# project-codeflare/instaslice

Measured on NVIDIA B200. Metric: placements_per_sec, higher is better.
Workload: dtype u8

## Files before the change

instaslice_b200/csrc/isl_kernels.cuh:

```cuda
#pragma once

#include <cuda_runtime.h>
#include <stdint.h>

#include "../../include/islplace.h"

namespace isl {

constexpr uint32_t kChunk = 65536;
constexpr uint32_t kTile = 1024;
constexpr uint32_t kTileThreads = 256;
constexpr uint32_t kTilesPerChunk = kChunk / kTile;
constexpr uint32_t kQPad = 32;
constexpr uint32_t kQCap = kChunk + kQPad * ISL_MAX_PROFILES;
constexpr uint32_t kSweepThreads = 256;
constexpr uint32_t kSweepPerThread = 16;
constexpr uint32_t kSweepBlock = kSweepThreads * kSweepPerThread;
constexpr uint32_t kSkip = 0xFFu;
constexpr uint32_t kInf = 0xFFFFFFFFu;
constexpr uint32_t kMaxCand = ISL_MAX_PROFILES * ISL_MAX_STARTS;
constexpr uint32_t kChainThreads = 256;
constexpr uint32_t kMaxTables = ISL_MAX_TABLES;

#ifndef ISL_UNIFORM_WARP
// ... 871 lines not shown
    asm volatile("ld.relaxed.gpu.global.u64 %0, [%1];" : "=l"(v) : "l"(p) : "memory");
    return v;
}
__device__ __forceinline__ void st_relaxed_gpu_u64(unsigned long long* p, unsigned long long v) {
    asm volatile("st.relaxed.gpu.global.u64 [%0], %1;" ::"l"(p), "l"(v) : "memory");
}
__device__ __forceinline__ unsigned long long ld_relaxed_sys_u64(const unsigned long long* p) {
    unsigned long long v;
    asm volatile("ld.relaxed.sys.global.u64 %0, [%1];" : "=l"(v) : "l"(p) : "memory");
    return v;
}
__device__ __forceinline__ void st_relaxed_sys_u64(unsigned long long* p, unsigned long long v) {
    asm volatile("st.relaxed.sys.global.u64 [%0], %1;" ::"l"(p), "l"(v) : "memory");
}

__device__ __forceinline__ uint32_t spec_spread_warp(uint32_t h, uint32_t qc, uint32_t w, uint32_t members, int d, bool weighted, uint32_t lane) {
    const bool in = (members >> lane) & 1u;
    if (!weighted) w = 1;
    const uint32_t light = __ballot_sync(0xFFFFFFFFu, in && w <= 1), heavy = __ballot_sync(0xFFFFFFFFu, in && w > 1);
    const uint32_t tot = __reduce_add_sync(0xFFFFFFFFu, in ? qc * w : 0u);
    if (d == 0 || members == 0) return h;
    const uint32_t last = 31u - __clz(light ? light : heavy);
    int dp = in && lane != last && tot ? __float2int_rn((float)d * (float)qc / (float)tot) : 0;
    const int used = __reduce_add_sync(0xFFFFFFFFu, dp * (int)w);
    const int wl = (int)__shfl_sync(0xFFFFFFFFu, w, last);
    if (lane == last) dp = (d - used) / wl;
    if (!in) return h;
    const int v = (int)h + dp;
    return (uint32_t)(v < 0 ? 0 : (v > (int)qc ? (int)qc : v));
}

__device__ __forceinline__ uint32_t lds_u32(uint32_t sa) { uint32_t v; asm volatile("ld.shared.u32 %0, [%1];" : "=r"(v) : "r"(sa)); return v; }
__device__ __forceinline__ uint32_t lds_u16(uint32_t sa) { uint32_t v; asm volatile("ld.shared.u16 %0, [%1];" : "=r"(v) : "r"(sa)); return v; }
__device__ __forceinline__ void sts_v2_if(bool pred, uint32_t sa, uint32_t x, uint32_t y) {
    asm volatile("{ .reg .pred p; setp.ne.u32 p, %0, 0; @p st.shared.v2.u32 [%1], {%2, %3}; }" ::"r"((uint32_t)pred), "r"(sa), "r"(x), "r"(y) : "memory");
}
__device__ __forceinline__ uint32_t add_if(bool pred, uint32_t x, uint32_t inc) {
    asm volatile("{ .reg .pred p; setp.ne.u32 p, %1, 0; @p add.u32 %0, %0, %2; }" : "+r"(x) : "r"((uint32_t)pred), "r"(inc));
    return x;
}
__device__ __forceinline__ uint32_t redux_min_u32(uint32_t v) {
// ... 21 lines not shown
template <int K, bool kP15, bool kSpec>
__global__ void __launch_bounds__(kPipeThreads, 1) k_pipeline(CandTab tab, PipeArgs a) {
    extern __shared__ __align__(16) uint8_t smem[];
    uint32_t* s_occ32 = reinterpret_cast<uint32_t*>(smem);
    uint32_t* s_cand = reinterpret_cast<uint32_t*>(smem + kPipeOffCand);
    uint2* s_log = reinterpret_cast<uint2*>(smem + kPipeOffLog);
    __shared__ uint16_t s_feas[kMaxTables * 256];
    __shared__ uint8_t s_tab[kSegMax * kSubMax];
    __shared__ uint32_t s_heads[ISL_MAX_PROFILES], s_wn[ISL_MAX_PROFILES], s_wbase[ISL_MAX_PROFILES], s_qbeg[ISL_MAX_PROFILES], s_pop[ISL_MAX_PROFILES];
    __shared__ uint32_t s_maxacc[ISL_MAX_PROFILES], s_minsize[ISL_MAX_PROFILES], s_usable[kMaxTables], s_plist[ISL_MAX_PROFILES], s_nplist;
    __shared__ uint32_t s_warp[kPipeThreads / 32], s_ncand, s_nfree, s_nlog, s_idle, s_closed;
    __shared__ uint32_t s_specH[ISL_MAX_PROFILES], s_specX[ISL_MAX_PROFILES], s_specXp[ISL_MAX_PROFILES], s_qc[ISL_MAX_PROFILES];
    __shared__ uint32_t s_acc[4], s_grp_big, s_grp_small, s_specflag, s_bigd[32], s_nbigd, s_dqr[2], s_us[kMaxTables], s_qo[ISL_MAX_PROFILES];
    __shared__ uint8_t s_smallm[kMaxTables][ISL_MAX_PROFILES];
    __shared__ uint32_t s_wlo[ISL_MAX_PROFILES], s_wlen[ISL_MAX_PROFILES], s_woff[ISL_MAX_PROFILES], s_wvalid, s_restage;
    __shared__ uint32_t s_predc, s_predA[ISL_MAX_PROFILES], s_predB[ISL_MAX_PROFILES], s_havepred;
    __shared__ uint32_t s_Hc[ISL_MAX_PROFILES], s_Xc[ISL_MAX_PROFILES], s_capst[3], s_cap, s_capped;
    const uint32_t tid = threadIdx.x, lane = tid & 31u, warp = tid >> 5, seg = blockIdx.x;
    if (seg == a.n_seg) {
        __shared__ uint32_t s_stop;
        for (uint32_t c = 0; c < a.n_chunks; ++c) {
            if (tid == 0) {
                uint32_t stop = 0;
                const unsigned long long t0 = globaltimer_ns();
                while (ld_acquire_gpu(a.done_cnt + c) < a.n_seg) {
                    if (a.ready && ld_acquire_gpu(a.ready + (a.open ? c : a.chunks[c].batch)) == ~a.epoch) { stop = 1; break; }
                    __nanosleep(256);
                    if (globaltimer_ns() - t0 > a.wait_ns + 5000000000ull) __trap();
                }
                s_stop = stop;
            }
// ... 188 lines not shown
        auto pub_down = [&](unsigned long long* p, unsigned long long v) {
            st_relaxed_gpu_u64(p, v);
            if (xr) for (uint32_t r = a.spec_rank + 1; r < a.spec_world; ++r) st_relaxed_sys_u64(a.spec_peer[r] + (p - a.spec_mem), v);
        };
        auto pub_nb = [&](unsigned long long* p, unsigned long long v, bool prev) {
            const bool remote = xr && (prev ? (seg == 0 && a.spec_rank > 0) : (seg + 1 == a.n_seg && a.spec_rank + 1 < a.spec_world));
            if (remote) st_relaxed_sys_u64(a.spec_peer[prev ? a.spec_rank - 1 : a.spec_rank + 1] + (p - a.spec_mem), v);
            else st_relaxed_gpu_u64(p, v);
        };
        if (spec) {
            uint16_t* s_mj = reinterpret_cast<uint16_t*>(s_wkey);
            if (tid < ISL_MAX_PROFILES) {
                const bool on = ((active >> tid) & 1u) && s_maxacc[tid] != 0 && cc->qcnt[tid] != 0;
                s_qc[tid] = on ? cc->qcnt[tid] : 0u; s_qo[tid] = cc->qoff[tid];
                const uint32_t big = __ballot_sync(0xFFFFu, on && s_minsize[tid] >= 4), small = __ballot_sync(0xFFFFu, on && s_minsize[tid] < 4);
                if (tid == 0) { s_grp_big = big; s_grp_small = small; s_acc[0] = 0; s_acc[1] = 0; s_acc[2] = 0; }
                if (tid < kMaxTables) { uint32_t us = 0; for (uint32_t m = small; m; m &= m - 1) us |= s_smallm[tid][__ffs(m) - 1]; s_us[tid] = us; }
            }
            __syncthreads();
            {
                constexpr uint32_t kGpt = kSegMax / kPipeThreads;
                const uint32_t gb = s_grp_big, nb = s_nbigd;
                uint32_t mq = 0, mw = 0, mo = 0;
#pragma unroll
                for (uint32_t x = 0; x < kGpt; ++x) {
                    const uint32_t g = kGpt * tid + x;
                    if (g < n_sb) {
                        const uint32_t t = s_tab[sb_base + g], o0 = reinterpret_cast<const uint8_t*>(s_occ32)[sb_base + g], us = s_us[t];
                        uint32_t o = o0;
                        for (uint32_t it = 0; it < 2; ++it) {
                            uint32_t best = 0;
                            for (uint32_t y = 0; y < nb; ++y) {
// ... 34 lines not shown
                uint32_t ql = 0;
                for (uint32_t x = 0; x < kPer; ++x) { const uint32_t j = lane * kPer + x; if (j < gseg) ql += s_mj[j]; }
                uint32_t incl = ql;
#pragma unroll
                for (int d = 1; d < 32; d <<= 1) { const uint32_t t = __shfl_up_sync(0xFFFFFFFFu, incl, d); if ((int)lane >= d) incl += t; }
                uint32_t run = incl - ql, r = 0;
                for (uint32_t x = 0; x < kPer; ++x) {
                    const uint32_t j = lane * kPer + x;
                    if (j < gseg) { r += run < totb ? s_mj[kSpecStride + j] : s_mj[2 * kSpecStride + j]; run += s_mj[j]; }
                }
                r = __reduce_add_sync(0xFFFFFFFFu, r);
                const uint32_t Q = min(__shfl_sync(0xFFFFFFFFu, incl, 31), totb), R = min(r, tots);
                {
                    const uint32_t qcl = lane < ISL_MAX_PROFILES ? s_qc[lane] : 0u, wl = lane < ISL_MAX_PROFILES ? s_minsize[lane] : 1u;
                    uint32_t hg = lane < ISL_MAX_PROFILES && gseg == 0 && a.heads_in ? a.heads_in[(size_t)c * ISL_MAX_PROFILES + lane] : 0u;
                    if (gseg > 0) {
                        hg = spec_spread_warp(hg, qcl, wl, s_grp_big, (int)Q, false, lane);
                        hg = spec_spread_warp(hg, qcl, wl, s_grp_small, (int)R, true, lane);
                    }
                    if (lane < ISL_MAX_PROFILES) s_specH[lane] = hg;
                }
            }
            __syncthreads();
        }
        uint32_t rnd = 1;
        bool c_prev = spec ? gseg == 0 : seg == 0, need_sim = true, idle_break = false;
        bool known_exact = gseg == 0;
        if (tid == 0) { s_capst[0] = 0; s_capst[1] = 0; s_capst[2] = 0; s_cap = kLogCap + 1; s_capped = 0; s_wvalid = 0; s_havepred = 0; }
        bool p_final = false; unsigned long long p_word = 0;
        const unsigned long long t_cell = tr && spec ? globaltimer_ns() : 0ull, sims_cell = st_sims;
#ifdef ISL_SPEC_DBG_STAMPS
        unsigned long long* dbg = a.spec_dbg && a.spec_dbg_cell == ((c << 16) | seg) ? a.spec_dbg : nullptr;
#else
        constexpr unsigned long long* dbg = nullptr;
#endif
        while (true) {
        stamp_if(dbg && tid == 0, dbg + rnd * 8 + 0);
        if (need_sim) {
        asm volatile("cp.async.wait_group 0;" ::: "memory");
        if (tid < 32) {
            uint32_t h = 0, wn = 0, left = 0;
            bool from_done = false;
            const uint32_t tag = a.epoch & 0x7FFFu;
            stamp_if(tr && tid == 0, tr + 0);
            if (spec) {
                if (tid < ISL_MAX_PROFILES) h = s_specH[tid];
            } else if (sb > 0) {
                if (tid < ISL_MAX_PROFILES) h = s_heads[tid] + s_pop[tid];
            } else if (seg > 0) {
                const uint32_t* pt = a.tokens + (tok_chunk + seg - 1) * kTokStride + (tid & 15u);
                const uint32_t* pd = a.tokens + (tok_chunk + a.n_seg) * kTokStride + (tid & 15u);
                bool ok = tid >= ISL_MAX_PROFILES;
// ... 11 lines not shown
                const unsigned long long t0 = globaltimer_ns();
                while (!__all_sync(0xFFFFFFFFu, ok)) {
                    if (!ok) {
                        const uint32_t v = ld_relaxed_sys(slot);
                        if ((v >> 17) == xtag) { h = v & 0x1FFFFu; ok = true; }
                        else if (globaltimer_ns() - t0 > a.wait_ns) __trap();
                    }
                }
                if (tid < ISL_MAX_PROFILES) st_relaxed_sys(slot, 0u);
            } else if (tid < ISL_MAX_PROFILES) h = a.heads_in ? a.heads_in[(size_t)c * ISL_MAX_PROFILES + tid] : 0u;
            stamp_if(tr && tid == 0, tr + 1);
            const bool all_done = sb == 0 && __all_sync(0xFFFFFFFFu, from_done || tid >= ISL_MAX_PROFILES);
            if (tid < ISL_MAX_PROFILES) {
                const uint32_t qc = spec ? s_qc[tid] : cc->qcnt[tid], qo = spec ? s_qo[tid] : cc->qoff[tid];
                left = ((active >> tid) & 1u) && qc > h ? qc - h : 0u;
                wn = min(left, min(s_ncand * s_maxacc[tid], s_nfree / s_minsize[tid]));
                s_heads[tid] = h; s_pop[tid] = 0;
                if (!kSpec) {
                    s_wn[tid] = wn;
                    s_qbeg[tid] = qo + h;
                }
            }
            bool win_keep = true;
            if (kSpec) {
                uint32_t lo = 0, len = 0, woff = 0;
                bool ok = true;
                const uint32_t qc = tid < ISL_MAX_PROFILES ? s_qc[tid] : 0u;
                if (tid < ISL_MAX_PROFILES) {
                    lo = s_wlo[tid]; len = s_wlen[tid];
                    if (left == 0) woff = len;
                    else { ok = s_wvalid && h >= lo && (h + wn + 2 <= lo + len || lo + len >= qc); woff = h - lo; }
// ... 16 lines not shown
                if (kSpec) {
                    s_restage = win_keep ? 0u : 1u;
                    if (!win_keep) s_wvalid = idle ? 0u : 1u;
                }
                s_cap = spec && s_capst[1] && !known_exact ? min(kLogCap + 1, ((s_capst[0] * 21u) >> 4) + 64u) : kLogCap + 1;
                s_capped = 0;
            }
            uint32_t incl = wn + kWinPad;
#pragma unroll
            for (int d = 1; d < 16; d <<= 1) { const uint32_t t = __shfl_up_sync(0xFFFFFFFFu, incl, d); if ((int)lane >= d) incl += t; }
            if (tid < ISL_MAX_PROFILES) s_wbase[tid] = incl - (wn + kWinPad);
        }
        __syncthreads();
        stamp_if(tr && tid == 0, tr + 8);
        stamp_if(dbg && tid == 0, dbg + rnd * 8 + 1);
        if (s_idle && spec) { if (tid == 0) { s_nlog = 0; spec_steps = 0; spec_visited = 0; } }
        else if (s_idle) {
            if (warp == 0) {
                const bool last = seg == a.n_seg - 1;
                uint32_t* tok = a.tokens + (tok_chunk + seg) * kTokStride;
                uint32_t* peer = last && a.outbox ? a.outbox + (size_t)c * kTokStride : nullptr;
                if (lane < ISL_MAX_PROFILES) {
                    const uint32_t h = s_heads[lane];
                    st_relaxed_gpu(tok + lane, ((a.epoch & 0x7FFFu) << 17) | h);
                    if (last && a.heads_out) a.heads_out[(size_t)c * ISL_MAX_PROFILES + lane] = h;
                    if (peer) st_relaxed_sys(peer + lane, ((a.xepoch % 32767u + 1u) << 17) | h);
                }
                __syncwarp();
                if (lane == 0) {
                    if (tr) { tr[2] = globaltimer_ns(); tr[3] = tr[2]; }
// ... 3 lines not shown
            idle_break = true;
            break;
        }
        if (!s_idle) {
        {
            const uint32_t npl = kSpec && !s_restage ? 0u : s_nplist;
            const uint16_t* __restrict__ sq = reinterpret_cast<const uint16_t*>(smem + kPipeOffQ);
            for (uint32_t x = 0; x < npl; ++x) {
                const uint32_t p = s_plist[x], wn = kSpec ? s_wlen[p] : s_wn[p], pk = p << 11, qb = s_qbeg[p];
                uint32_t* __restrict__ dst = s_wkey + s_wbase[p];
                for (uint32_t i = tid; i < wn + kWinPad; i += kPipeThreads) { const uint32_t v = sq[qb + min(i, wn)]; dst[i] = i < wn ? (v << 15) | pk : kInf; }
            }
            stamp_if(tr && tid == 0, tr + 10);
            store_if(tr && tid == 0, tr + 11, s_wn[s_plist[0]] | ((unsigned long long)s_nfree << 32));
        }
        __syncthreads();
        stamp_if(tr && tid == 0, tr + 9);
        if (is_chain_warp(warp)) {
            const uint32_t n_cand = s_ncand;
            uint32_t tcur[K], tnext[K], tnn[K], wa[K], wa0[K];
#pragma unroll
            for (int k = 0; k < K; ++k) {
                wa0[k] = sa_wkey + 4 * (s_wbase[cprof[k]] + (kSpec ? s_woff[cprof[k]] : 0u));
                const bool has = valid[k];
                tcur[k] = has ? lds_u32(wa0[k]) | klow[k] : kInf;
                tnext[k] = has ? lds_u32(wa0[k] + 4) | klow[k] : kInf;
                const bool two = has && s_wn[cprof[k]] >= 1;
                tnn[k] = two ? lds_u32(wa0[k] + 8) : kInf;
                wa[k] = wa0[k] + 12;
            }
            uint32_t la = sa_log, ca = sa_cand + 8;
            uint32_t z0[K], z1[K], z2[K], g1[K], g2[K], cm8[K];
// ... 114 lines not shown
            const bool last = seg == a.n_seg - 1;
            uint32_t* peer = last && a.outbox ? a.outbox + (size_t)c * kTokStride : nullptr;
            if (last_sub && lane < ISL_MAX_PROFILES && !spec) {
                const uint32_t h = s_heads[lane] + s_pop[lane];
                st_relaxed_gpu(tok + lane, ((a.epoch & 0x7FFFu) << 17) | h);
                if (last && a.heads_out) a.heads_out[(size_t)c * ISL_MAX_PROFILES + lane] = h;
                if (peer) st_relaxed_sys(peer + lane, ((a.xepoch % 32767u + 1u) << 17) | h);
            }
            __syncwarp();
            if (lane == 0) {
                s_nlog = nlog;
                s_capped = cut ? 1u : 0u;
                if (tr) tr[2] = globaltimer_ns();
            }
        }
        else if (spec && tid == kPipeThreads - 32 && rnd >= 3 && gseg + 1 < gtot) {
            const unsigned long long t0 = globaltimer_ns();
            uint32_t spins = 0;
            while (true) {
                const unsigned long long w = sld(sm.ack + gseg + 1);
                if ((uint32_t)(w >> 32) == tage && (uint32_t)w + 2u >= rnd) break;
                if ((++spins & 255u) == 0 && globaltimer_ns() - t0 > a.wait_ns) __trap();
            }
        }
        }
        __syncthreads();
        }
        if (!spec) break;
        {
            const unsigned long long tagr = tagb | ((unsigned long long)rnd << 32);
            if (tid < 32) {
                uint32_t X = 0, dq = 0, dr = 0, pop = 0;
                const bool was_cut = s_capped != 0;
                if (tid < ISL_MAX_PROFILES) { pop = s_pop[tid]; X = s_heads[tid] + pop; }
                if (was_cut) {
                    int eq = 0, er = 0;
                    uint32_t xe = 0;
                    const uint32_t qcl = tid < ISL_MAX_PROFILES ? s_qc[tid] : 0u, wl = tid < ISL_MAX_PROFILES ? s_minsize[tid] : 1u;
                    if (tid < ISL_MAX_PROFILES) {
                        const int d = (int)s_heads[tid] - (int)s_Hc[tid];
                        if ((s_grp_big >> tid) & 1u) eq = d;
                        if ((s_grp_small >> tid) & 1u) er = d * (int)s_minsize[tid];
                        xe = s_Xc[tid];
                    }
                    eq = __reduce_add_sync(0xFFFFFFFFu, eq); er = __reduce_add_sync(0xFFFFFFFFu, er);
                    xe = spec_spread_warp(xe, qcl, wl, s_grp_big, eq, false, lane);
                    xe = spec_spread_warp(xe, qcl, wl, s_grp_small, er, true, lane);
                    if (tid < ISL_MAX_PROFILES) { X = max(xe, s_heads[tid]); pop = X - s_heads[tid]; }
                }
                if (tid < ISL_MAX_PROFILES) {
                    s_specX[tid] = X;
                    if (!was_cut) { s_Hc[tid] = s_heads[tid]; s_Xc[tid] = X; }
                    if ((s_grp_big >> tid) & 1u) dq = pop;
                    if ((s_grp_small >> tid) & 1u) dr = pop * s_minsize[tid];
                }
                if (tid == 0) { if (was_cut) s_capst[2] = 0; else { s_capst[0] = max(s_capst[0], s_nlog); s_capst[1] = 1; s_capst[2] = 1; } }
                dq = __reduce_add_sync(0xFFFFFFFFu, dq); dr = __reduce_add_sync(0xFFFFFFFFu, dr);
                if (rnd >= 3 && gseg + 1 < gtot && !(need_sim && !s_idle)) {
                    const unsigned long long t0 = globaltimer_ns();
                    uint32_t spins = 0;
                    while (true) {
                        const unsigned long long w = sld(sm.ack + gseg + 1);
                        if ((uint32_t)(w >> 32) == tage && (uint32_t)w + 2u >= rnd) break;
                        if ((++spins & 255u) == 0 && globaltimer_ns() - t0 > a.wait_ns) __trap();
                    }
                }
                if (tid < ISL_MAX_PROFILES) pub_nb(sm.x + ((size_t)gseg * 2 + (rnd & 1u)) * 16 + tid, tagr | X, false);
                if (tid == 16) pub_down(sm.d + (size_t)rnd * kSpecStride + gseg, tagr | ((c_prev ? 1u : 0u) << 31) | (dq << 13) | dr);
                if (tid == 0) { s_dqr[0] = dq; s_dqr[1] = dr; s_acc[0] = 0; s_acc[1] = 0; }
                stamp_if(dbg && tid == 0, dbg + rnd * 8 + 4);
            }
            __syncthreads();
            bool cbit = true;
            if (tid < gseg) {
                unsigned long long w = p_word;
                if (!p_final) {
                    const unsigned long long t0 = globaltimer_ns();
                    uint32_t spins = 0;
                    while (true) {
                        w = sld(sm.d + (size_t)rnd * kSpecStride + tid);
                        if ((w >> 32) == (tagr >> 32)) { cbit = (w >> 31) & 1u; break; }
                        if ((spins++ & 3u) == 0) {
                            w = sld(sm.df + tid);
                            if ((w >> 32) == (tagF >> 32) && ((w >> 24) & 0xFFu) <= rnd) { p_final = true; p_word = w; break; }
                        }
                        if ((spins & 255u) == 0 && globaltimer_ns() - t0 > a.wait_ns) __trap();
                    }
                }
                atomicAdd(&s_acc[0], (uint32_t)(w >> 13) & 0x7FFu);
                atomicAdd(&s_acc[1], (uint32_t)w & 0x1FFFu);
            }
            if (gseg > 0 && tid >= 192 && tid < 192 + ISL_MAX_PROFILES) {
                const uint32_t i = tid - 192;
                unsigned long long w = p_word;
                if (!p_final) {
                    const unsigned long long t0 = globaltimer_ns();
                    uint32_t spins = 0;
                    while (true) {
                        w = sld(sm.x + ((size_t)(gseg - 1) * 2 + (rnd & 1u)) * 16 + i);
                        if ((w >> 32) == (tagr >> 32)) break;
                        if ((spins++ & 3u) == 0) {
                            w = sld(sm.xf + (size_t)(gseg - 1) * 16 + i);
                            if ((w >> 32) == (tagF >> 32) && ((w >> 24) & 0xFFu) <= rnd) { p_final = true; p_word = w; break; }
                        }
                        if ((spins & 255u) == 0 && globaltimer_ns() - t0 > a.wait_ns) __trap();
                    }
                }
                s_specXp[i] = (uint32_t)w & 0x1FFFFu;
            }
            if (tid + 1 == gseg) s_predc = cbit ? 1u : 0u;
            const int unset = __syncthreads_count(!cbit);
            const bool allc = unset == 0;
            const bool near = allc || (unset == 1 && !s_predc);
            const bool certified = allc && c_prev;
            stamp_if(dbg && tid == 0, dbg + rnd * 8 + 5);
            store_if(dbg && tid == 0, dbg + rnd * 8 + 7, s_nlog | ((unsigned long long)need_sim << 32));
            if (gseg > 0 && tid == 192) pub_nb(sm.ack + gseg, ((unsigned long long)tage << 32) | (certified ? 0xFFFFu : rnd), true);
            if (certified) {
                if (tid < ISL_MAX_PROFILES) {
                    pub_nb(sm.xf + (size_t)gseg * 16 + tid, tagF | (rnd << 24) | s_specX[tid], false);
                    if (gseg == gtot - 1 && a.heads_out) a.heads_out[(size_t)c * ISL_MAX_PROFILES + tid] = s_specX[tid];
                }
                if (tid == 16) pub_down(sm.df + gseg, tagF | (rnd << 24) | (s_dqr[0] << 13) | s_dqr[1]);
                if (tid == 0) { st_steps += spec_steps; st_visited += spec_visited; if (gseg == gtot - 1) { st_rounds_sum += rnd; ++st_cells; } if (tr) { tr[0] = t_cell; tr[2] = globaltimer_ns(); tr[6] = s_nlog; tr[7] = st_sims - sims_cell; tr[11] = rnd; } }
                break;
            }
            if (tid < 32) {
                const bool same = tid >= ISL_MAX_PROFILES || s_specH[tid] == s_specXp[tid];
                const bool cnow = __all_sync(0xFFFFFFFFu, same);
                uint32_t mq = 0, mr = 0, hold = 0, hn = 0;
                const uint32_t qcl = tid < ISL_MAX_PROFILES ? s_qc[tid] : 0u, wl = tid < ISL_MAX_PROFILES ? s_minsize[tid] : 1u;
                if (tid < ISL_MAX_PROFILES) {
                    hold = s_specH[tid];
                    hn = s_specXp[tid];
                    if ((s_grp_big >> tid) & 1u) mq = hn;
                    if ((s_grp_small >> tid) & 1u) mr = hn * s_minsize[tid];
                }
                mq = __reduce_add_sync(0xFFFFFFFFu, mq); mr = __reduce_add_sync(0xFFFFFFFFu, mr);
                hn = spec_spread_warp(hn, qcl, wl, s_grp_big, (int)s_acc[0] - (int)mq, false, lane);
                hn = spec_spread_warp(hn, qcl, wl, s_grp_small, (int)s_acc[1] - (int)mr, true, lane);
                {
                    const uint32_t xp = tid < ISL_MAX_PROFILES ? s_specXp[tid] : 0u;
                    uint32_t ea = 0, eb = 0;
                    if (tid < ISL_MAX_PROFILES && s_havepred) { ea = (uint32_t)abs((int)s_predA[tid] - (int)xp); eb = (uint32_t)abs((int)s_predB[tid] - (int)xp); }
                    ea = __reduce_add_sync(0xFFFFFFFFu, ea); eb = __reduce_add_sync(0xFFFFFFFFu, eb);
                    __syncwarp();
                    if (tid < ISL_MAX_PROFILES) { s_predA[tid] = hn; s_predB[tid] = xp; }
                    if (tid == 0 && rnd >= 2) s_havepred = 1;
                    if (eb < ea) hn = xp;
                }
                if (tid < ISL_MAX_PROFILES) s_specH[tid] = hn;
                const bool moved = tid < ISL_MAX_PROFILES && hn != hold;
                const bool changed = __any_sync(0xFFFFFFFFu, moved);
                if (tid == 0) s_specflag = (cnow && s_capst[2] ? 1u : 0u) | (changed || !s_capst[2] ? 2u : 0u);
                stamp_if(dbg && tid == 0, dbg + rnd * 8 + 6);
            }
            __syncthreads();
            c_prev = s_specflag & 1u; need_sim = s_specflag & 2u; known_exact = near;
            if (++rnd >= kSpecRounds - 1) __trap();
        }
        }
        if (idle_break) break;
        if (last_sub && c + 1 < a.n_chunks && !a.ready && !a.window) { queue_load_async(c + 1); prefetched = true; }
        {
            const uint32_t nlog = s_nlog;
            for (uint32_t j = tid; j < nlog; j += kPipeThreads) {
                const uint2 e = s_log[j];
                const uint32_t l = sb_base + (s_cand[((e.y - sa_cand) >> 2) - 2] >> 16), mask = e.x & 0xFFu, t = (e.x >> 15) & 0xFFFFu;
                const uint2 rec = pack_result(flip_gpu(lo_s + l, a.flip), __ffs(mask) - 1, __popc(mask), ISL_ST_PLACED);
                a.out[cd.req_off + t] = rec;
                if (a.owner_out) a.owner_out[cd.req_off + t] = rec;
                atomicOr(&s_occ32[l >> 2], mask << ((l & 3u) * 8u));
            }
// ... 153 lines not shown
```

instaslice_b200/csrc/islplace.cu:

```cuda
#include <algorithm>
#include <atomic>
#include <cstdio>
#include <cstdlib>
#include <cstring>
#include <cmath>
#include <mutex>
#include <new>
#include <vector>

#include "isl_kernels.cuh"

using namespace isl;

static constexpr uint32_t kMaxStreamChunks = 4096;

struct isl_engine {
    isl_config cfg{};
    int device = 0;
    cudaStream_t stream = nullptr;
    bool own_stream = false;
    std::mutex mu;
    char cuda_err[256] = {0};

    DevProfiles prof{};
// ... 40 lines not shown
    uint32_t* d_inbox = nullptr;
    uint32_t* d_outbox = nullptr;
    bool has_prev = false, outbox_local = false;
    unsigned long long* d_trace = nullptr; uint32_t cap_trace = 0, trace_chunks = 0, trace_seg = 0;
    int max_coresident = 0;
    cudaStream_t feed_stream = nullptr; cudaEvent_t ev_feed = nullptr, ev_feed_done = nullptr;
    uint32_t* d_ready = nullptr; uint32_t cap_ready = 0;
    uint32_t* d_done_cnt = nullptr; uint32_t cap_done = 0;
    uint8_t* d_occ_snap = nullptr; size_t snap_bytes = 0; uint32_t snap_G = 0;
    bool delivered = false;
    size_t scratch_bytes = 0;
    unsigned long long wait_ns = 20000000000ull;
    uint32_t window = 0;
    uint32_t spec_mode = ISL_SPEC_AUTO;
    unsigned long long* d_specdbg = nullptr;
    unsigned long long* spec_peer[8] = {}; bool spec_peer_local = false, spec_shared = false;
    uint32_t spec_world = 0, spec_rank = 0, spec_bounds[9] = {};
    unsigned long long* d_spec = nullptr; uint32_t cap_spec = 0, spec_hi = 0;
    struct Open {
        bool active = false, launched = false;
        uint32_t max_batches = 0, submitted = 0, epoch = 0, seg = 0, n_seg = 0, sub = 0, q_stride = 0, free_stride = 0, tiles_per_batch = 0;
        bool spec = false;
        uint32_t* h_done = nullptr; uint32_t* d_done_host = nullptr; uint32_t cap_done = 0;
        ChunkDesc* h_chunks = nullptr; TileDesc* h_tiles = nullptr; uint32_t cap_desc = 0;
    } open;
    uint2* d_owner_out = nullptr; bool owner_local = false;
    uint32_t ring_world = 0;

    isl_stats st{};
    cudaEvent_t ev[6] = {nullptr, nullptr, nullptr, nullptr, nullptr, nullptr};
// ... 454 lines not shown
        ISL_CUDA(e, cudaMemsetAsync(e->d_trace, 0, (size_t)n_chunks * n_seg * kTraceWords * sizeof(unsigned long long), e->stream));
        e->trace_chunks = n_chunks; e->trace_seg = n_seg;
    }
    args.trace = (e->cfg.flags & ISL_FLAG_TRACE) ? e->d_trace : nullptr;
    args.inbox = ring && e->has_prev ? e->d_inbox : nullptr; args.outbox = ring ? e->d_outbox : nullptr; args.xepoch = xepoch;
    if (spec) {
        if (int rc2 = prepare_spec(e, n_chunks, epoch, e->stream)) return rc2;
        args.spec = getenv("ISL_SPEC_NOREUSE") ? 3u : 1u; args.spec_mem = e->d_spec; args.spec_total = n_seg;
        if (ring) {
            args.inbox = nullptr; args.outbox = nullptr;
            args.spec_world = e->spec_world; args.spec_rank = e->spec_rank; args.spec_base = e->lo / seg; args.spec_total = ceil_div(e->G, seg);
            for (uint32_t r = 0; r < e->spec_world; ++r) args.spec_peer[r] = e->spec_peer[r];
        }
        if (const char* v = getenv("ISL_SPEC_DBG")) {
            unsigned cchunk = 0, cstage = 0;
            if (sscanf(v, "%u,%u", &cchunk, &cstage) == 2) {
                if (!e->d_specdbg) ISL_CUDA(e, cudaMalloc(&e->d_specdbg, kSpecRounds * 8 * sizeof(unsigned long long)));
                ISL_CUDA(e, cudaMemsetAsync(e->d_specdbg, 0, kSpecRounds * 8 * sizeof(unsigned long long), e->stream));
                args.spec_dbg = e->d_specdbg; args.spec_dbg_cell = (cchunk << 16) | cstage;
            }
        }
    }
    int rc;
    const bool p15 = e->prof.n == ISL_MAX_PROFILES;
    switch (e->n_cand_slots) {
        case 1: rc = p15 ? launch_pipeline<1, true>(e, args) : launch_pipeline<1, false>(e, args); break;
        case 2: rc = p15 ? launch_pipeline<2, true>(e, args) : launch_pipeline<2, false>(e, args); break;
        default: rc = p15 ? launch_pipeline<4, true>(e, args) : launch_pipeline<4, false>(e, args); break;
    }
    if (rc == ISL_ESTATE && ring) return ISL_ERANGE;
    if (rc == ISL_ESTATE) {
        e->max_coresident = -1;
        if (feed) {
            ISL_CUDA(e, cudaEventRecord(e->ev_feed_done, pre));
// ... 753 lines not shown
}

int isl_set_causal_window(isl_engine* e, uint32_t window) {
    if (!e) return ISL_EINVAL;
    if (e->open.active) return ISL_ESTATE;
    std::lock_guard<std::mutex> lk(e->mu);
    e->window = window;
    return ISL_OK;
}

int isl_debug_spec_rounds(isl_engine* e, uint64_t* out, uint32_t max_words) {
    if (!e || !out || !e->d_specdbg) return ISL_EINVAL;
    std::lock_guard<std::mutex> lk(e->mu);
    DeviceGuard guard(e->device);
    ISL_CUDA(e, cudaStreamSynchronize(e->stream));
    ISL_CUDA(e, cudaMemcpy(out, e->d_specdbg, std::min<size_t>(max_words, kSpecRounds * 8) * sizeof(uint64_t), cudaMemcpyDeviceToHost));
    return ISL_OK;
}

int isl_set_speculation(isl_engine* e, uint32_t mode) {
    if (!e || mode > ISL_SPEC_ON) return ISL_EINVAL;
    if (e->open.active) return ISL_ESTATE;
    std::lock_guard<std::mutex> lk(e->mu);
    e->spec_mode = mode;
    return ISL_OK;
}

int isl_set_ring_world(isl_engine* e, uint32_t world) {
    if (!e) return ISL_EINVAL;
    std::lock_guard<std::mutex> lk(e->mu);
    e->ring_world = world;
// ... 222 lines not shown
```

Measured before the change: 140.0 million.

## Overlap speculative neighbor polling with chain work and drop block barriers

```diff
diff --git a/instaslice_b200/csrc/isl_kernels.cuh b/instaslice_b200/csrc/isl_kernels.cuh
--- a/instaslice_b200/csrc/isl_kernels.cuh
+++ b/instaslice_b200/csrc/isl_kernels.cuh
@@ -909,17 +909,24 @@
     asm volatile("st.relaxed.sys.global.u64 [%0], %1;" ::"l"(p), "l"(v) : "memory");
 }
 
-__device__ __forceinline__ uint32_t spec_spread_warp(uint32_t h, uint32_t qc, uint32_t w, uint32_t members, int d, bool weighted, uint32_t lane) {
+struct SpreadK { uint32_t tot, last; int wl; };
+__device__ __forceinline__ SpreadK spec_spread_prep(uint32_t qc, uint32_t w, uint32_t members, bool weighted, uint32_t lane) {
     const bool in = (members >> lane) & 1u;
     if (!weighted) w = 1;
     const uint32_t light = __ballot_sync(0xFFFFFFFFu, in && w <= 1), heavy = __ballot_sync(0xFFFFFFFFu, in && w > 1);
-    const uint32_t tot = __reduce_add_sync(0xFFFFFFFFu, in ? qc * w : 0u);
+    SpreadK k;
+    k.tot = __reduce_add_sync(0xFFFFFFFFu, in ? qc * w : 0u);
+    k.last = 31u - __clz(light ? light : heavy);
+    k.wl = (int)__shfl_sync(0xFFFFFFFFu, w, k.last);
+    return k;
+}
+__device__ __forceinline__ uint32_t spec_spread_warp(uint32_t h, uint32_t qc, uint32_t w, uint32_t members, int d, bool weighted, const SpreadK& k, uint32_t lane) {
+    const bool in = (members >> lane) & 1u;
+    if (!weighted) w = 1;
     if (d == 0 || members == 0) return h;
-    const uint32_t last = 31u - __clz(light ? light : heavy);
-    int dp = in && lane != last && tot ? __float2int_rn((float)d * (float)qc / (float)tot) : 0;
+    int dp = in && lane != k.last && k.tot ? __float2int_rn((float)d * (float)qc / (float)k.tot) : 0;
     const int used = __reduce_add_sync(0xFFFFFFFFu, dp * (int)w);
-    const int wl = (int)__shfl_sync(0xFFFFFFFFu, w, last);
-    if (lane == last) dp = (d - used) / wl;
+    if (lane == k.last) dp = (d - used) / k.wl;
     if (!in) return h;
     const int v = (int)h + dp;
     return (uint32_t)(v < 0 ? 0 : (v > (int)qc ? (int)qc : v));
@@ -971,7 +978,11 @@
     __shared__ uint32_t s_acc[4], s_grp_big, s_grp_small, s_specflag, s_bigd[32], s_nbigd, s_dqr[2], s_us[kMaxTables], s_qo[ISL_MAX_PROFILES];
     __shared__ uint8_t s_smallm[kMaxTables][ISL_MAX_PROFILES];
     __shared__ uint32_t s_wlo[ISL_MAX_PROFILES], s_wlen[ISL_MAX_PROFILES], s_woff[ISL_MAX_PROFILES], s_wvalid, s_restage;
-    __shared__ uint32_t s_predc, s_predA[ISL_MAX_PROFILES], s_predB[ISL_MAX_PROFILES], s_havepred;
+    __shared__ uint32_t s_predA[ISL_MAX_PROFILES], s_predB[ISL_MAX_PROFILES], s_havepred;
+    __shared__ uint32_t s_ackd;
+    __shared__ uint32_t s_ngot, s_nun, s_pbad;
+    __shared__ SpreadK s_spk[2];
+    __shared__ uint32_t s_wcap[ISL_MAX_PROFILES];
     __shared__ uint32_t s_Hc[ISL_MAX_PROFILES], s_Xc[ISL_MAX_PROFILES], s_capst[3], s_cap, s_capped;
     const uint32_t tid = threadIdx.x, lane = tid & 31u, warp = tid >> 5, seg = blockIdx.x;
     if (seg == a.n_seg) {
@@ -1190,8 +1201,9 @@
                 const bool on = ((active >> tid) & 1u) && s_maxacc[tid] != 0 && cc->qcnt[tid] != 0;
                 s_qc[tid] = on ? cc->qcnt[tid] : 0u; s_qo[tid] = cc->qoff[tid];
                 const uint32_t big = __ballot_sync(0xFFFFu, on && s_minsize[tid] >= 4), small = __ballot_sync(0xFFFFu, on && s_minsize[tid] < 4);
-                if (tid == 0) { s_grp_big = big; s_grp_small = small; s_acc[0] = 0; s_acc[1] = 0; s_acc[2] = 0; }
+                if (tid == 0) { s_grp_big = big; s_grp_small = small; s_acc[0] = 0; s_acc[1] = 0; s_acc[2] = 0; s_ackd = 0; }
                 if (tid < kMaxTables) { uint32_t us = 0; for (uint32_t m = small; m; m &= m - 1) us |= s_smallm[tid][__ffs(m) - 1]; s_us[tid] = us; }
+                s_wcap[tid] = min(s_ncand * s_maxacc[tid], s_nfree / s_minsize[tid]);
             }
             __syncthreads();
             {
@@ -1256,9 +1268,11 @@
                 {
                     const uint32_t qcl = lane < ISL_MAX_PROFILES ? s_qc[lane] : 0u, wl = lane < ISL_MAX_PROFILES ? s_minsize[lane] : 1u;
                     uint32_t hg = lane < ISL_MAX_PROFILES && gseg == 0 && a.heads_in ? a.heads_in[(size_t)c * ISL_MAX_PROFILES + lane] : 0u;
+                    const SpreadK kb = spec_spread_prep(qcl, wl, s_grp_big, false, lane), ks = spec_spread_prep(qcl, wl, s_grp_small, true, lane);
+                    if (lane == 0) { s_spk[0] = kb; s_spk[1] = ks; s_acc[0] = 0; s_acc[1] = 0; s_ngot = 0; s_nun = 0; s_pbad = 0; }
                     if (gseg > 0) {
-                        hg = spec_spread_warp(hg, qcl, wl, s_grp_big, (int)Q, false, lane);
-                        hg = spec_spread_warp(hg, qcl, wl, s_grp_small, (int)R, true, lane);
+                        hg = spec_spread_warp(hg, qcl, wl, s_grp_big, (int)Q, false, kb, lane);
+                        hg = spec_spread_warp(hg, qcl, wl, s_grp_small, (int)R, true, ks, lane);
                     }
                     if (lane < ISL_MAX_PROFILES) s_specH[lane] = hg;
                 }
@@ -1276,8 +1290,16 @@
 #else
         constexpr unsigned long long* dbg = nullptr;
 #endif
+#ifdef ISL_SPEC_PHASE_STAMPS
+#define ISL_PHASE(pred, i) stamp_if(kSpec && (pred) && a.spec_dbg, a.spec_dbg + (((size_t)c * kSpecStride + gseg) * kSpecRounds + rnd) * 8 + (i))
+#define ISL_PHASE_WORD(pred, v) store_if(kSpec && (pred) && a.spec_dbg, a.spec_dbg + (((size_t)c * kSpecStride + gseg) * kSpecRounds + rnd) * 8 + 7, (v))
+#else
+#define ISL_PHASE(pred, i) ((void)0)
+#define ISL_PHASE_WORD(pred, v) ((void)0)
+#endif
         while (true) {
         stamp_if(dbg && tid == 0, dbg + rnd * 8 + 0);
+        ISL_PHASE(tid == 32, 0);
         if (need_sim) {
         asm volatile("cp.async.wait_group 0;" ::: "memory");
         if (tid < 32) {
@@ -1319,7 +1341,7 @@
             if (tid < ISL_MAX_PROFILES) {
                 const uint32_t qc = spec ? s_qc[tid] : cc->qcnt[tid], qo = spec ? s_qo[tid] : cc->qoff[tid];
                 left = ((active >> tid) & 1u) && qc > h ? qc - h : 0u;
-                wn = min(left, min(s_ncand * s_maxacc[tid], s_nfree / s_minsize[tid]));
+                wn = min(left, kSpec ? s_wcap[tid] : min(s_ncand * s_maxacc[tid], s_nfree / s_minsize[tid]));
                 s_heads[tid] = h; s_pop[tid] = 0;
                 if (!kSpec) {
                     s_wn[tid] = wn;
@@ -1366,6 +1388,7 @@
         __syncthreads();
         stamp_if(tr && tid == 0, tr + 8);
         stamp_if(dbg && tid == 0, dbg + rnd * 8 + 1);
+        ISL_PHASE(tid == 32, 1);
         if (s_idle && spec) { if (tid == 0) { s_nlog = 0; spec_steps = 0; spec_visited = 0; } }
         else if (s_idle) {
             if (warp == 0) {
@@ -1399,8 +1422,9 @@
             stamp_if(tr && tid == 0, tr + 10);
             store_if(tr && tid == 0, tr + 11, s_wn[s_plist[0]] | ((unsigned long long)s_nfree << 32));
         }
-        __syncthreads();
+        if (!kSpec || s_restage) __syncthreads();
         stamp_if(tr && tid == 0, tr + 9);
+        ISL_PHASE(tid == 32, 2);
         if (is_chain_warp(warp)) {
             const uint32_t n_cand = s_ncand;
             uint32_t tcur[K], tnext[K], tnn[K], wa[K], wa0[K];
@@ -1545,7 +1569,11 @@
                 if (tr) tr[2] = globaltimer_ns();
             }
         }
-        else if (spec && tid == kPipeThreads - 32 && rnd >= 3 && gseg + 1 < gtot) {
+        }
+        if (!kSpec) __syncthreads();
+        ISL_PHASE(tid == 0, 3);
+        }
+        if (spec && tid == kPipeThreads - 32 && rnd >= 3 && gseg + 1 < gtot) {
             const unsigned long long t0 = globaltimer_ns();
             uint32_t spins = 0;
             while (true) {
@@ -1553,9 +1581,36 @@
                 if ((uint32_t)(w >> 32) == tage && (uint32_t)w + 2u >= rnd) break;
                 if ((++spins & 255u) == 0 && globaltimer_ns() - t0 > a.wait_ns) __trap();
             }
-        }
-        }
-        __syncthreads();
+            __threadfence_block();
+            *reinterpret_cast<volatile uint32_t*>(&s_ackd) = rnd;
+        }
+        if (spec && ((tid >= 32 && tid < 32 + gseg) || (gseg > 0 && tid >= 192 && tid < 192 + ISL_MAX_PROFILES))) {
+            const unsigned long long tagr = tagb | ((unsigned long long)rnd << 32);
+            const bool dw = tid < 192;
+            const uint32_t j = dw ? tid - 32 : tid - 192;
+            unsigned long long w = p_word;
+            if (!p_final) {
+                const unsigned long long t0 = globaltimer_ns();
+                uint32_t spins = 0;
+                while (true) {
+                    w = sld(dw ? sm.d + (size_t)rnd * kSpecStride + j : sm.x + ((size_t)(gseg - 1) * 2 + (rnd & 1u)) * 16 + j);
+                    if ((w >> 32) == (tagr >> 32)) break;
+                    if ((spins++ & 3u) == 0) {
+                        w = sld(dw ? sm.df + j : sm.xf + (size_t)(gseg - 1) * 16 + j);
+                        if ((w >> 32) == (tagF >> 32) && ((w >> 24) & 0xFFu) <= rnd) { p_final = true; p_word = w; w |= 1ull << 31; break; }
+                    }
+                    if ((spins & 255u) == 0 && globaltimer_ns() - t0 > a.wait_ns) __trap();
+                }
+            }
+            if (dw) {
+                atomicAdd(&s_acc[0], (uint32_t)(w >> 13) & 0x7FFu);
+                atomicAdd(&s_acc[1], (uint32_t)w & 0x1FFFu);
+                if (!p_final && !((w >> 31) & 1u)) { atomicAdd(&s_nun, 1u); if (j + 1 == gseg) s_pbad = 1; }
+            } else {
+                s_specXp[j] = (uint32_t)w & 0x1FFFFu;
+            }
+            __threadfence_block();
+            atomicAdd(&s_ngot, 1u);
         }
         if (!spec) break;
         {
@@ -1575,8 +1630,8 @@
                         xe = s_Xc[tid];
                     }
                     eq = __reduce_add_sync(0xFFFFFFFFu, eq); er = __reduce_add_sync(0xFFFFFFFFu, er);
-                    xe = spec_spread_warp(xe, qcl, wl, s_grp_big, eq, false, lane);
-                    xe = spec_spread_warp(xe, qcl, wl, s_grp_small, er, true, lane);
+                    xe = spec_spread_warp(xe, qcl, wl, s_grp_big, eq, false, s_spk[0], lane);
+                    xe = spec_spread_warp(xe, qcl, wl, s_grp_small, er, true, s_spk[1], lane);
                     if (tid < ISL_MAX_PROFILES) { X = max(xe, s_heads[tid]); pop = X - s_heads[tid]; }
                 }
                 if (tid < ISL_MAX_PROFILES) {
@@ -1587,107 +1642,78 @@
                 }
                 if (tid == 0) { if (was_cut) s_capst[2] = 0; else { s_capst[0] = max(s_capst[0], s_nlog); s_capst[1] = 1; s_capst[2] = 1; } }
                 dq = __reduce_add_sync(0xFFFFFFFFu, dq); dr = __reduce_add_sync(0xFFFFFFFFu, dr);
-                if (rnd >= 3 && gseg + 1 < gtot && !(need_sim && !s_idle)) {
-                    const unsigned long long t0 = globaltimer_ns();
-                    uint32_t spins = 0;
-                    while (true) {
-                        const unsigned long long w = sld(sm.ack + gseg + 1);
-                        if ((uint32_t)(w >> 32) == tage && (uint32_t)w + 2u >= rnd) break;
-                        if ((++spins & 255u) == 0 && globaltimer_ns() - t0 > a.wait_ns) __trap();
-                    }
+                if (rnd >= 3 && gseg + 1 < gtot) {
+                    while (!__all_sync(0xFFFFFFFFu, *reinterpret_cast<volatile uint32_t*>(&s_ackd) >= rnd)) {}
+                    __threadfence_block();
                 }
                 if (tid < ISL_MAX_PROFILES) pub_nb(sm.x + ((size_t)gseg * 2 + (rnd & 1u)) * 16 + tid, tagr | X, false);
                 if (tid == 16) pub_down(sm.d + (size_t)rnd * kSpecStride + gseg, tagr | ((c_prev ? 1u : 0u) << 31) | (dq << 13) | dr);
-                if (tid == 0) { s_dqr[0] = dq; s_dqr[1] = dr; s_acc[0] = 0; s_acc[1] = 0; }
+                if (tid == 0) { s_dqr[0] = dq; s_dqr[1] = dr; }
                 stamp_if(dbg && tid == 0, dbg + rnd * 8 + 4);
+                ISL_PHASE(tid == 0, 4);
+                {
+                    const uint32_t expect = gseg + (gseg > 0 ? ISL_MAX_PROFILES : 0u);
+                    while (!__all_sync(0xFFFFFFFFu, *reinterpret_cast<volatile uint32_t*>(&s_ngot) >= expect)) {}
+                    __threadfence_block();
+                }
+                const uint32_t unset = *reinterpret_cast<volatile uint32_t*>(&s_nun);
+                const bool predbad = *reinterpret_cast<volatile uint32_t*>(&s_pbad) != 0;
+                ISL_PHASE(tid == 0, 5);
+                ISL_PHASE_WORD(tid == 0, s_nlog | ((unsigned long long)need_sim << 32));
+                const bool allc = unset == 0;
+                known_exact = allc || (unset == 1 && predbad);
+                const bool certified = allc && c_prev;
+                stamp_if(dbg && tid == 0, dbg + rnd * 8 + 5);
+                store_if(dbg && tid == 0, dbg + rnd * 8 + 7, s_nlog | ((unsigned long long)need_sim << 32));
+                if (gseg > 0 && tid == 0) pub_nb(sm.ack + gseg, ((unsigned long long)tage << 32) | (certified ? 0xFFFFu : rnd), true);
+                if (certified) {
+                    if (tid < ISL_MAX_PROFILES) {
+                        pub_nb(sm.xf + (size_t)gseg * 16 + tid, tagF | (rnd << 24) | s_specX[tid], false);
+                        if (gseg == gtot - 1 && a.heads_out) a.heads_out[(size_t)c * ISL_MAX_PROFILES + tid] = s_specX[tid];
+                    }
+                    if (tid == 16) pub_down(sm.df + gseg, tagF | (rnd << 24) | (s_dqr[0] << 13) | s_dqr[1]);
+                    if (tid == 0) {
+                        st_steps += spec_steps; st_visited += spec_visited; if (gseg == gtot - 1) { st_rounds_sum += rnd; ++st_cells; }
+                        if (tr) { tr[0] = t_cell; tr[2] = globaltimer_ns(); tr[6] = s_nlog; tr[7] = st_sims - sims_cell; tr[11] = rnd; }
+                        s_specflag = 4u;
+                    }
+                } else {
+                    const bool same = tid >= ISL_MAX_PROFILES || s_specH[tid] == s_specXp[tid];
+                    const bool cnow = __all_sync(0xFFFFFFFFu, same);
+                    uint32_t mq = 0, mr = 0, hold = 0, hn = 0;
+                    const uint32_t qcl = tid < ISL_MAX_PROFILES ? s_qc[tid] : 0u, wl = tid < ISL_MAX_PROFILES ? s_minsize[tid] : 1u;
+                    if (tid < ISL_MAX_PROFILES) {
+                        hold = s_specH[tid];
+                        hn = s_specXp[tid];
+                        if ((s_grp_big >> tid) & 1u) mq = hn;
+                        if ((s_grp_small >> tid) & 1u) mr = hn * s_minsize[tid];
+                    }
+                    mq = __reduce_add_sync(0xFFFFFFFFu, mq); mr = __reduce_add_sync(0xFFFFFFFFu, mr);
+                    hn = spec_spread_warp(hn, qcl, wl, s_grp_big, (int)s_acc[0] - (int)mq, false, s_spk[0], lane);
+                    hn = spec_spread_warp(hn, qcl, wl, s_grp_small, (int)s_acc[1] - (int)mr, true, s_spk[1], lane);
+                    {
+                        const uint32_t xq = tid < ISL_MAX_PROFILES ? s_specXp[tid] : 0u;
+                        uint32_t ea = 0, eb = 0;
+                        if (tid < ISL_MAX_PROFILES && s_havepred) { ea = (uint32_t)abs((int)s_predA[tid] - (int)xq); eb = (uint32_t)abs((int)s_predB[tid] - (int)xq); }
+                        ea = __reduce_add_sync(0xFFFFFFFFu, ea); eb = __reduce_add_sync(0xFFFFFFFFu, eb);
+                        __syncwarp();
+                        if (tid < ISL_MAX_PROFILES) { s_predA[tid] = hn; s_predB[tid] = xq; }
+                        if (tid == 0 && rnd >= 2) s_havepred = 1;
+                        if (eb < ea) hn = xq;
+                    }
+                    if (tid < ISL_MAX_PROFILES) s_specH[tid] = hn;
+                    const bool moved = tid < ISL_MAX_PROFILES && hn != hold;
+                    const bool changed = __any_sync(0xFFFFFFFFu, moved);
+                    if (tid == 0) s_specflag = (cnow && s_capst[2] ? 1u : 0u) | (changed || !s_capst[2] ? 2u : 0u);
+                    stamp_if(dbg && tid == 0, dbg + rnd * 8 + 6);
+                }
+                __syncwarp();
+                if (tid == 0) { s_acc[0] = 0; s_acc[1] = 0; s_ngot = 0; s_nun = 0; s_pbad = 0; }
             }
             __syncthreads();
-            bool cbit = true;
-            if (tid < gseg) {
-                unsigned long long w = p_word;
-                if (!p_final) {
-                    const unsigned long long t0 = globaltimer_ns();
-                    uint32_t spins = 0;
-                    while (true) {
-                        w = sld(sm.d + (size_t)rnd * kSpecStride + tid);
-                        if ((w >> 32) == (tagr >> 32)) { cbit = (w >> 31) & 1u; break; }
-                        if ((spins++ & 3u) == 0) {
-                            w = sld(sm.df + tid);
-                            if ((w >> 32) == (tagF >> 32) && ((w >> 24) & 0xFFu) <= rnd) { p_final = true; p_word = w; break; }
-                        }
-                        if ((spins & 255u) == 0 && globaltimer_ns() - t0 > a.wait_ns) __trap();
-                    }
-                }
-                atomicAdd(&s_acc[0], (uint32_t)(w >> 13) & 0x7FFu);
-                atomicAdd(&s_acc[1], (uint32_t)w & 0x1FFFu);
-            }
-            if (gseg > 0 && tid >= 192 && tid < 192 + ISL_MAX_PROFILES) {
-                const uint32_t i = tid - 192;
-                unsigned long long w = p_word;
-                if (!p_final) {
-                    const unsigned long long t0 = globaltimer_ns();
-                    uint32_t spins = 0;
-                    while (true) {
-                        w = sld(sm.x + ((size_t)(gseg - 1) * 2 + (rnd & 1u)) * 16 + i);
-                        if ((w >> 32) == (tagr >> 32)) break;
-                        if ((spins++ & 3u) == 0) {
-                            w = sld(sm.xf + (size_t)(gseg - 1) * 16 + i);
-                            if ((w >> 32) == (tagF >> 32) && ((w >> 24) & 0xFFu) <= rnd) { p_final = true; p_word = w; break; }
-                        }
-                        if ((spins & 255u) == 0 && globaltimer_ns() - t0 > a.wait_ns) __trap();
-                    }
-                }
-                s_specXp[i] = (uint32_t)w & 0x1FFFFu;
-            }
-            if (tid + 1 == gseg) s_predc = cbit ? 1u : 0u;
-            const int unset = __syncthreads_count(!cbit);
-            const bool allc = unset == 0;
-            const bool near = allc || (unset == 1 && !s_predc);
-            const bool certified = allc && c_prev;
-            stamp_if(dbg && tid == 0, dbg + rnd * 8 + 5);
-            store_if(dbg && tid == 0, dbg + rnd * 8 + 7, s_nlog | ((unsigned long long)need_sim << 32));
-            if (gseg > 0 && tid == 192) pub_nb(sm.ack + gseg, ((unsigned long long)tage << 32) | (certified ? 0xFFFFu : rnd), true);
-            if (certified) {
-                if (tid < ISL_MAX_PROFILES) {
-                    pub_nb(sm.xf + (size_t)gseg * 16 + tid, tagF | (rnd << 24) | s_specX[tid], false);
-                    if (gseg == gtot - 1 && a.heads_out) a.heads_out[(size_t)c * ISL_MAX_PROFILES + tid] = s_specX[tid];
-                }
-                if (tid == 16) pub_down(sm.df + gseg, tagF | (rnd << 24) | (s_dqr[0] << 13) | s_dqr[1]);
-                if (tid == 0) { st_steps += spec_steps; st_visited += spec_visited; if (gseg == gtot - 1) { st_rounds_sum += rnd; ++st_cells; } if (tr) { tr[0] = t_cell; tr[2] = globaltimer_ns(); tr[6] = s_nlog; tr[7] = st_sims - sims_cell; tr[11] = rnd; } }
-                break;
-            }
-            if (tid < 32) {
-                const bool same = tid >= ISL_MAX_PROFILES || s_specH[tid] == s_specXp[tid];
-                const bool cnow = __all_sync(0xFFFFFFFFu, same);
-                uint32_t mq = 0, mr = 0, hold = 0, hn = 0;
-                const uint32_t qcl = tid < ISL_MAX_PROFILES ? s_qc[tid] : 0u, wl = tid < ISL_MAX_PROFILES ? s_minsize[tid] : 1u;
-                if (tid < ISL_MAX_PROFILES) {
-                    hold = s_specH[tid];
-                    hn = s_specXp[tid];
-                    if ((s_grp_big >> tid) & 1u) mq = hn;
-                    if ((s_grp_small >> tid) & 1u) mr = hn * s_minsize[tid];
-                }
-                mq = __reduce_add_sync(0xFFFFFFFFu, mq); mr = __reduce_add_sync(0xFFFFFFFFu, mr);
-                hn = spec_spread_warp(hn, qcl, wl, s_grp_big, (int)s_acc[0] - (int)mq, false, lane);
-                hn = spec_spread_warp(hn, qcl, wl, s_grp_small, (int)s_acc[1] - (int)mr, true, lane);
-                {
-                    const uint32_t xp = tid < ISL_MAX_PROFILES ? s_specXp[tid] : 0u;
-                    uint32_t ea = 0, eb = 0;
-                    if (tid < ISL_MAX_PROFILES && s_havepred) { ea = (uint32_t)abs((int)s_predA[tid] - (int)xp); eb = (uint32_t)abs((int)s_predB[tid] - (int)xp); }
-                    ea = __reduce_add_sync(0xFFFFFFFFu, ea); eb = __reduce_add_sync(0xFFFFFFFFu, eb);
-                    __syncwarp();
-                    if (tid < ISL_MAX_PROFILES) { s_predA[tid] = hn; s_predB[tid] = xp; }
-                    if (tid == 0 && rnd >= 2) s_havepred = 1;
-                    if (eb < ea) hn = xp;
-                }
-                if (tid < ISL_MAX_PROFILES) s_specH[tid] = hn;
-                const bool moved = tid < ISL_MAX_PROFILES && hn != hold;
-                const bool changed = __any_sync(0xFFFFFFFFu, moved);
-                if (tid == 0) s_specflag = (cnow && s_capst[2] ? 1u : 0u) | (changed || !s_capst[2] ? 2u : 0u);
-                stamp_if(dbg && tid == 0, dbg + rnd * 8 + 6);
-            }
-            __syncthreads();
-            c_prev = s_specflag & 1u; need_sim = s_specflag & 2u; known_exact = near;
+            ISL_PHASE(tid == 32, 6);
+            if (s_specflag & 4u) break;
+            c_prev = s_specflag & 1u; need_sim = s_specflag & 2u;
             if (++rnd >= kSpecRounds - 1) __trap();
         }
         }
diff --git a/instaslice_b200/csrc/islplace.cu b/instaslice_b200/csrc/islplace.cu
--- a/instaslice_b200/csrc/islplace.cu
+++ b/instaslice_b200/csrc/islplace.cu
@@ -78,6 +78,7 @@
     uint32_t window = 0;
     uint32_t spec_mode = ISL_SPEC_AUTO;
     unsigned long long* d_specdbg = nullptr;
+    size_t n_specdbg = 0;
     unsigned long long* spec_peer[8] = {}; bool spec_peer_local = false, spec_shared = false;
     uint32_t spec_world = 0, spec_rank = 0, spec_bounds[9] = {};
     unsigned long long* d_spec = nullptr; uint32_t cap_spec = 0, spec_hi = 0;
@@ -562,10 +563,16 @@
         }
         if (const char* v = getenv("ISL_SPEC_DBG")) {
             unsigned cchunk = 0, cstage = 0;
-            if (sscanf(v, "%u,%u", &cchunk, &cstage) == 2) {
-                if (!e->d_specdbg) ISL_CUDA(e, cudaMalloc(&e->d_specdbg, kSpecRounds * 8 * sizeof(unsigned long long)));
-                ISL_CUDA(e, cudaMemsetAsync(e->d_specdbg, 0, kSpecRounds * 8 * sizeof(unsigned long long), e->stream));
-                args.spec_dbg = e->d_specdbg; args.spec_dbg_cell = (cchunk << 16) | cstage;
+            const bool phases = strcmp(v, "phases") == 0;
+            if (phases || sscanf(v, "%u,%u", &cchunk, &cstage) == 2) {
+                const size_t words = phases ? (size_t)n_chunks * kSpecStride * kSpecRounds * 8 : (size_t)kSpecRounds * 8;
+                if (words > e->n_specdbg) {
+                    cudaFree(e->d_specdbg); e->d_specdbg = nullptr; e->n_specdbg = 0;
+                    ISL_CUDA(e, cudaMalloc(&e->d_specdbg, words * sizeof(unsigned long long)));
+                    e->n_specdbg = words;
+                }
+                ISL_CUDA(e, cudaMemsetAsync(e->d_specdbg, 0, words * sizeof(unsigned long long), e->stream));
+                args.spec_dbg = e->d_specdbg; args.spec_dbg_cell = phases ? 0xFFFFFFFFu : (cchunk << 16) | cstage;
             }
         }
     }
@@ -1349,7 +1356,7 @@
     std::lock_guard<std::mutex> lk(e->mu);
     DeviceGuard guard(e->device);
     ISL_CUDA(e, cudaStreamSynchronize(e->stream));
-    ISL_CUDA(e, cudaMemcpy(out, e->d_specdbg, std::min<size_t>(max_words, kSpecRounds * 8) * sizeof(uint64_t), cudaMemcpyDeviceToHost));
+    ISL_CUDA(e, cudaMemcpy(out, e->d_specdbg, std::min<size_t>(max_words, e->n_specdbg) * sizeof(uint64_t), cudaMemcpyDeviceToHost));
     return ISL_OK;
 }
 
```

Result: faster. 142.3 million, median of 6 (+1.6%).
